# dRaniwal/RAJNI-ViT

Hardware: AMD Instinct MI355X
Metric: images/sec ViT-B/16@224 with README schedule (higher is better)
Workload: dtype bf16

## Files before the change

### rajni-vit_amd/csrc/attention.hip

```cpp
#include "common.h"

namespace {

constexpr int AT_THREADS = 256;
constexpr int AT_QROWS = 128;
constexpr int KV_CHUNK = 128;
constexpr int AT_LDS = 2 * KV_CHUNK * 128;

struct AttnArgs {
  const bf16_t* qkv;
  const int* idx;
  bf16_t* out;
  int n_src, np, H;
  int nq;
  float c;
  unsigned long long* stamps;
  unsigned char* out8;
  float oinv, oscale;
  float* row_scale;
};
__device__ __forceinline__ unsigned attn_pack4_e4m3(float a, float b, float c, float d) {
  a = __builtin_amdgcn_fmed3f(a, -448.f, 448.f); b = __builtin_amdgcn_fmed3f(b, -448.f, 448.f);
  c = __builtin_amdgcn_fmed3f(c, -448.f, 448.f); d = __builtin_amdgcn_fmed3f(d, -448.f, 448.f);
  int r = __builtin_amdgcn_cvt_pk_fp8_f32(a, b, 0, false);
  r = __builtin_amdgcn_cvt_pk_fp8_f32(c, d, r, true);
  return (unsigned)r;
}

__device__ __forceinline__ int k_off(int row, int chunk) {
  return row * 128 + ((chunk ^ ((row >> 1) & 7)) << 4);
}
__device__ __forceinline__ int v_off(int row, int chunk) {
  return row * 128 + ((chunk ^ (((row >> 1) & 1) << 2)) << 4);
}

__device__ __forceinline__ bf16x8 tr_pair(const char* sv, int row, int col) {
  typedef __attribute__((address_space(3))) s16x4* lds_s16x4;
  const int o0 = v_off(row, col >> 3) + (col & 7) * 2;
  const int o1 = v_off(row + 8, col >> 3) + (col & 7) * 2;
  const s16x4 lo = __builtin_amdgcn_ds_read_tr16_b64_v4i16((lds_s16x4)(sv + o0));
  const s16x4 hi = __builtin_amdgcn_ds_read_tr16_b64_v4i16((lds_s16x4)(sv + o1));
  typedef __attribute__((ext_vector_type(8))) short s16x8;
  const s16x8 v = {lo[0], lo[1], lo[2], lo[3], hi[0], hi[1], hi[2], hi[3]};
  return __builtin_bit_cast(bf16x8, v);
}

template <typename A = bf16_t>
__global__ void __launch_bounds__(AT_THREADS) attn_bf16_d64(const AttnArgs a) {
  __shared__ __attribute__((aligned(16))) char smem[AT_LDS];
  char* sk = smem;
  char* sv = smem + KV_CHUNK * 128;
  const int tid = threadIdx.x, wave = tid >> 6, lane = tid & 63;
  const int l31 = lane & 31, h = lane >> 5, g = lane >> 4, l15 = lane & 15;
  const int head = blockIdx.y, b = blockIdx.z;
  const int np = a.np, C = a.H * 64, C3 = 3 * C;
  const bf16_t* img = a.qkv + (long)b * a.n_src * C3;
  const int* idx = a.idx ? a.idx + (long)b * np : nullptr;

  const int qbase = blockIdx.x * AT_QROWS + wave * 32;
  const bool active = qbase < (a.nq < np ? a.nq : np);

  bf16x8 qf[4];
  {
    int q = qbase + l31;
    if (q > np - 1) q = np - 1;
    const int srow = idx ? idx[q] : q;
    const bf16_t* qp = img + (long)srow * C3 + head * 64 + 8 * h;
#pragma unroll
    for (int s = 0; s < 4; ++s) qf[s] = *reinterpret_cast<const bf16x8*>(qp + 16 * s);
  }

  f32x16 o0, o1;
#pragma unroll
  for (int r = 0; r < 16; ++r) { o0[r] = 0.f; o1[r] = 0.f; }
  float m_run = -INFINITY, l_run = 0.f;

  const int st_c = tid & 7, st_r = tid >> 3;

  for (int c0 = 0; c0 < np; c0 += KV_CHUNK) {
    uint4 kreg[4], vreg[4];
#pragma unroll
    for (int i = 0; i < 4; ++i) {
      const int t = c0 + st_r + 32 * i;
      if (t < np) {
        const int srow = idx ? idx[t] : t;
        const bf16_t* rp = img + (long)srow * C3 + head * 64 + st_c * 8;
        kreg[i] = *reinterpret_cast<const uint4*>(rp + C);
        vreg[i] = *reinterpret_cast<const uint4*>(rp + 2 * C);
      } else {
        kreg[i] = make_uint4(0, 0, 0, 0);
        vreg[i] = make_uint4(0, 0, 0, 0);
      }
    }
    __syncthreads();
#pragma unroll
    for (int i = 0; i < 4; ++i) {
      const int row = st_r + 32 * i;
      *reinterpret_cast<uint4*>(sk + k_off(row, st_c)) = kreg[i];
      *reinterpret_cast<uint4*>(sv + v_off(row, st_c)) = vreg[i];
    }
    __syncthreads();

    if (active) {
      const int nsub = (np - c0 + 31) >> 5;
      for (int kb = 0; kb < 4 && kb < nsub; ++kb) {
        f32x16 s;
#pragma unroll
        for (int r = 0; r < 16; ++r) s[r] = 0.f;
        const int krow = kb * 32 + l31;
#pragma unroll
        for (int ks = 0; ks < 4; ++ks) {
          const bf16x8 kf = *reinterpret_cast<const bf16x8*>(sk + k_off(krow, 2 * ks + h));
          s = mfma_32x32x16<A>(kf, qf[ks], s);
        }
        const int nvalid = np - c0 - kb * 32;
        if (nvalid < 32) {
#pragma unroll
          for (int r = 0; r < 16; ++r) {
            const int kr = (r & 3) + 8 * (r >> 2) + 4 * h;
            if (kr >= nvalid) s[r] = -INFINITY;
          }
        }
        float mx = s[0];
#pragma unroll
        for (int r = 1; r < 16; ++r) mx = fmaxf(mx, s[r]);
        mx = fmaxf(mx, __shfl_xor(mx, 32, 64));
        const float mxc = mx * a.c;
        if (__builtin_amdgcn_ballot_w64(mxc > m_run + 8.0f) != 0) {
          const float m_new = fmaxf(m_run, mxc);
          const float alpha = __builtin_amdgcn_exp2f(m_run - m_new);
          l_run *= alpha;
          m_run = m_new;
#pragma unroll
          for (int r = 0; r < 16; ++r) { o0[r] *= alpha; o1[r] *= alpha; }
        }
        float p[16];
        float lsum = 0.f;
#pragma unroll
        for (int r = 0; r < 16; ++r) {
          p[r] = __builtin_amdgcn_exp2f(fmaf(s[r], a.c, -m_run));
          lsum += p[r];
        }
        l_run += lsum;
        bf16x8 pb[2];
#pragma unroll
        for (int s2 = 0; s2 < 2; ++s2) {
          typedef __attribute__((ext_vector_type(4))) unsigned u32x4;
          const u32x4 w = {pack2<A>(p[8 * s2 + 0], p[8 * s2 + 1]), pack2<A>(p[8 * s2 + 2], p[8 * s2 + 3]),
                           pack2<A>(p[8 * s2 + 4], p[8 * s2 + 5]), pack2<A>(p[8 * s2 + 6], p[8 * s2 + 7])};
          pb[s2] = __builtin_bit_cast(bf16x8, w);
        }
#pragma unroll
        for (int s2 = 0; s2 < 2; ++s2) {
          const int key0 = kb * 32 + 16 * s2 + 4 * h + (l15 >> 2);
          const int col = 16 * (g & 1) + 4 * (l15 & 3);
          const bf16x8 v0 = tr_pair(sv, key0, col);
          const bf16x8 v1 = tr_pair(sv, key0, 32 + col);
          o0 = mfma_32x32x16<A>(v0, pb[s2], o0);
          o1 = mfma_32x32x16<A>(v1, pb[s2], o1);
        }
      }
    }
  }

  if (!active) return;
  const float l_tot = l_run + __shfl_xor(l_run, 32, 64);
  const float inv = 1.0f / l_tot;
  const int q = qbase + l31;
  if (q < np) {
    bf16_t* op = a.out + ((long)b * np + q) * C + head * 64 + 4 * h;
#pragma unroll
    for (int t = 0; t < 4; ++t) {
      uint2 w0, w1;
      w0.x = pack2<A>(o0[4 * t] * inv, o0[4 * t + 1] * inv);
      w0.y = pack2<A>(o0[4 * t + 2] * inv, o0[4 * t + 3] * inv);
      w1.x = pack2<A>(o1[4 * t] * inv, o1[4 * t + 1] * inv);
      w1.y = pack2<A>(o1[4 * t + 2] * inv, o1[4 * t + 3] * inv);
      *reinterpret_cast<uint2*>(op + 8 * t) = w0;
      *reinterpret_cast<uint2*>(op + 32 + 8 * t) = w1;
    }
  }
}


constexpr int ATF_THREADS = 512;
#ifndef RAJNI_ATTN_STAGE_MASK
#define RAJNI_ATTN_STAGE_MASK 0x78
#endif
constexpr bool stage_o(int nsub) { return (RAJNI_ATTN_STAGE_MASK >> (nsub - 1)) & 1; }

template <typename A, int NSUB, bool O8 = false>
__device__ __forceinline__ void attn_tile_compute(const char* sk, const char* sv, const bf16x8 (&qf)[4],
                                                  const AttnArgs& a, int b, int head, int qbase, int lane,
                                                  char* so = nullptr) {
  const int l31 = lane & 31, h = lane >> 5, g = lane >> 4, l15 = lane & 15;
  const int np = a.np, C = a.H * 64;
  f32x16 s[NSUB];
#pragma unroll
  for (int kb = 0; kb < NSUB; ++kb) {
#pragma unroll
    for (int r = 0; r < 16; ++r) s[kb][r] = 0.f;
    const int krow = kb * 32 + l31;
#pragma unroll
    for (int ks = 0; ks < 4; ++ks) {
      const bf16x8 kf = *reinterpret_cast<const bf16x8*>(sk + k_off(krow, 2 * ks + h));
      s[kb] = mfma_32x32x16<A>(kf, qf[ks], s[kb]);
    }
  }
#ifdef RAJNI_ATTN_STAMPS
  asm volatile("" :: "v"(s[0][0]), "v"(s[NSUB - 1][15]));
  const unsigned long long tsS = __builtin_amdgcn_s_memtime();
#endif
  {
    const int nvalid = np - (NSUB - 1) * 32;
    if (nvalid < 32) {
#pragma unroll
      for (int r = 0; r < 16; ++r) {
        const int kr = (r & 3) + 8 * (r >> 2) + 4 * h;
        if (kr >= nvalid) s[NSUB - 1][r] = -INFINITY;
      }
    }
  }
  float mx = s[0][0];
#pragma unroll
  for (int kb = 0; kb < NSUB; ++kb)
#pragma unroll
    for (int r = 0; r < 16; ++r) mx = fmaxf(mx, s[kb][r]);
  mx = fmaxf(mx, __shfl_xor(mx, 32, 64));
  const float mc = mx * a.c;
  float lsum = 0.f;
  f32x16 o0, o1;
#pragma unroll
  for (int r = 0; r < 16; ++r) { o0[r] = 0.f; o1[r] = 0.f; }
#pragma unroll
  for (int kb = 0; kb < NSUB; ++kb) {
    float p[16];
#pragma unroll
    for (int r = 0; r < 16; ++r) {
      p[r] = __builtin_amdgcn_exp2f(fmaf(s[kb][r], a.c, -mc));
      lsum += p[r];
    }
    bf16x8 pb[2];
#pragma unroll
    for (int s2 = 0; s2 < 2; ++s2) {
      typedef __attribute__((ext_vector_type(4))) unsigned u32x4;
      const u32x4 w = {pack2<A>(p[8 * s2 + 0], p[8 * s2 + 1]), pack2<A>(p[8 * s2 + 2], p[8 * s2 + 3]),
                       pack2<A>(p[8 * s2 + 4], p[8 * s2 + 5]), pack2<A>(p[8 * s2 + 6], p[8 * s2 + 7])};
      pb[s2] = __builtin_bit_cast(bf16x8, w);
    }
#pragma unroll
    for (int s2 = 0; s2 < 2; ++s2) {
      const int key0 = kb * 32 + 16 * s2 + 4 * h + (l15 >> 2);
      const int col = 16 * (g & 1) + 4 * (l15 & 3);
      const bf16x8 v0 = tr_pair(sv, key0, col);
      const bf16x8 v1 = tr_pair(sv, key0, 32 + col);
      o0 = mfma_32x32x16<A>(v0, pb[s2], o0);
      o1 = mfma_32x32x16<A>(v1, pb[s2], o1);
    }
  }
#ifdef RAJNI_ATTN_STAMPS
  asm volatile("" :: "v"(o0[0]), "v"(o1[15]));
  const unsigned long long tsP = __builtin_amdgcn_s_memtime();
  if (a.stamps != nullptr && qbase == 0 && lane == 0) {
    unsigned long long* o = a.stamps + ((size_t)b * a.H + head) * 8;
    o[1] = tsS; o[2] = tsP;
  }
#endif
  const float inv = 1.0f / (lsum + __shfl_xor(lsum, 32, 64));
  const int q = qbase + l31;
  __builtin_amdgcn_s_waitcnt(0x0F70);
  if constexpr (O8) {
    const float sc = inv * a.oinv;
    const int key = (l31 >> 2) & 3;
    char* wr = so + l31 * 64 + 4 * (h & 1);
#pragma unroll
    for (int t = 0; t < 4; ++t) {
      const unsigned w0 = attn_pack4_e4m3(o0[4 * t] * sc, o0[4 * t + 1] * sc, o0[4 * t + 2] * sc, o0[4 * t + 3] * sc);
      const unsigned w1 = attn_pack4_e4m3(o1[4 * t] * sc, o1[4 * t + 1] * sc, o1[4 * t + 2] * sc, o1[4 * t + 3] * sc);
      *reinterpret_cast<unsigned*>(wr + (((t >> 1) ^ key) << 4) + 8 * (t & 1)) = w0;
      *reinterpret_cast<unsigned*>(wr + (((2 + (t >> 1)) ^ key) << 4) + 8 * (t & 1)) = w1;
    }
    __builtin_amdgcn_fence(__ATOMIC_RELEASE, "wavefront");
    __builtin_amdgcn_wave_barrier();
    const int u = lane & 3;
    unsigned char* ob = a.out8 + ((long)b * np + qbase) * C + head * 64 + u * 16;
#pragma unroll
    for (int j = 0; j < 2; ++j) {
      const int r = (lane >> 2) + 16 * j;
      const uint4 v = *reinterpret_cast<const uint4*>(so + r * 64 + ((u ^ ((r >> 2) & 3)) << 4));
      if (qbase + r < np) *reinterpret_cast<uint4*>(ob + (long)r * C) = v;
    }
    if (head == 0 && h == 0 && q < np) a.row_scale[(long)b * np + q] = a.oscale;
    return;
  }
  if (so != nullptr) {
    const int key = (l31 ^ (l31 >> 3)) & 7;
    char* wr = so + l31 * 128 + 8 * h;
#pragma unroll
    for (int t = 0; t < 4; ++t) {
      uint2 w0, w1;
      w0.x = pack2<A>(o0[4 * t] * inv, o0[4 * t + 1] * inv);
      w0.y = pack2<A>(o0[4 * t + 2] * inv, o0[4 * t + 3] * inv);
      w1.x = pack2<A>(o1[4 * t] * inv, o1[4 * t + 1] * inv);
      w1.y = pack2<A>(o1[4 * t + 2] * inv, o1[4 * t + 3] * inv);
      *reinterpret_cast<uint2*>(wr + ((t ^ key) << 4)) = w0;
      *reinterpret_cast<uint2*>(wr + (((4 + t) ^ key) << 4)) = w1;
    }
    const int u = lane & 7;
    bf16_t* ob = a.out + ((long)b * np + qbase) * C + head * 64 + u * 8;
#pragma unroll
    for (int j = 0; j < 4; ++j) {
      const int r = (lane >> 3) + 8 * j;
      const uint4 v = *reinterpret_cast<const uint4*>(so + r * 128 + ((u ^ ((r ^ (r >> 3)) & 7)) << 4));
      if (qbase + r < np) *reinterpret_cast<uint4*>(ob + (long)r * C) = v;
    }
    return;
  }
  if (q < np) {
    bf16_t* op = a.out + ((long)b * np + q) * C + head * 64 + 4 * h;
#pragma unroll
    for (int t = 0; t < 4; ++t) {
      uint2 w0, w1;
      w0.x = pack2<A>(o0[4 * t] * inv, o0[4 * t + 1] * inv);
      w0.y = pack2<A>(o0[4 * t + 2] * inv, o0[4 * t + 3] * inv);
      w1.x = pack2<A>(o1[4 * t] * inv, o1[4 * t + 1] * inv);
      w1.y = pack2<A>(o1[4 * t + 2] * inv, o1[4 * t + 3] * inv);
      *reinterpret_cast<uint2*>(op + 8 * t) = w0;
      *reinterpret_cast<uint2*>(op + 32 + 8 * t) = w1;
    }
  }
}

template <int NSUB, typename A = bf16_t>
__global__ void __launch_bounds__(ATF_THREADS, 2) attn_bf16_d64_full(const AttnArgs a) {
  extern __shared__ __attribute__((aligned(16))) char smem[];
  constexpr int ROWS = NSUB * 32;
  char* sk = smem;
  char* sv = smem + ROWS * 128;
  const int tid = threadIdx.x, wave = tid >> 6, lane = tid & 63;
  const int l31 = lane & 31, h = lane >> 5, g = lane >> 4, l15 = lane & 15;
  const int head = blockIdx.x, b = blockIdx.y;
  const int np = a.np, C = a.H * 64, C3 = 3 * C;
  const bf16_t* img = a.qkv + (long)b * a.n_src * C3;
  const int* idx = a.idx ? a.idx + (long)b * np : nullptr;
  const int qbase = wave * 32;
  const bool active = qbase < (a.nq < np ? a.nq : np);

  bf16x8 qf[4];
  {
    int q = qbase + l31;
    if (q > np - 1) q = np - 1;
    const int srow = idx ? idx[q] : q;
    const bf16_t* qp = img + (long)srow * C3 + head * 64 + 8 * h;
#pragma unroll
    for (int s = 0; s < 4; ++s) qf[s] = *reinterpret_cast<const bf16x8*>(qp + 16 * s);
  }
  {
    const int st_c = tid & 7, st_r = tid >> 3;
#pragma unroll
    for (int i = 0; i < (ROWS + 63) / 64; ++i) {
      const int t = st_r + 64 * i;
      if (t < ROWS) {
        uint4 kr = make_uint4(0, 0, 0, 0), vr = make_uint4(0, 0, 0, 0);
        if (t < np) {
          const int srow = idx ? idx[t] : t;
          const bf16_t* rp = img + (long)srow * C3 + head * 64 + st_c * 8;
          kr = *reinterpret_cast<const uint4*>(rp + C);
          vr = *reinterpret_cast<const uint4*>(rp + 2 * C);
        }
        *reinterpret_cast<uint4*>(sk + k_off(t, st_c)) = kr;
        *reinterpret_cast<uint4*>(sv + v_off(t, st_c)) = vr;
      }
    }
  }
  __syncthreads();
  if (!active) return;
  attn_tile_compute<A, NSUB>(sk, sv, qf, a, b, head, qbase, lane);
}

__device__ __forceinline__ void dma16(const char* base, unsigned off, char* dst) {
  const unsigned lds = __builtin_amdgcn_readfirstlane((unsigned)(size_t)LDS_PTR(dst));
  unsigned keep;
  asm volatile("s_mov_b32 %0, m0\n\ts_mov_b32 m0, %2\n\ts_nop 0\n\tglobal_load_lds_dwordx4 %1, %3\n\ts_mov_b32 m0, %0"
               : "=&s"(keep) : "v"(off), "s"(lds), "s"(base) : "memory");
}

template <int NSUB, bool G, bool O8 = false, typename A = bf16_t>
__global__ void __launch_bounds__(ATF_THREADS, 2) attn_bf16_d64_stream(const AttnArgs a, int n_items) {
  extern __shared__ __attribute__((aligned(16))) char smem[];
  constexpr int ROWS = NSUB * 32, BUF = ROWS * 256, NP8 = ROWS / 8;
  constexpr bool STAGE_O = O8 || stage_o(NSUB);
  constexpr int STAGE_BYTES = O8 ? 2048 : 4096;
  constexpr int PER_WAVE = (NP8 + 7) / 8;
  const int tid = threadIdx.x, lane = tid & 63;
  const int wave = __builtin_amdgcn_readfirstlane(tid >> 6);
  const int l31 = lane & 31, h = lane >> 5;
  const int np = a.np, C = a.H * 64, C3 = 3 * C;
  const int qbase = wave * 32;
  const bool active = qbase < (a.nq < np ? a.nq : np);
  const int r_in = lane >> 3, pos = lane & 7;

  int trow[PER_WAVE];
#pragma unroll
  for (int i = 0; i < PER_WAVE; ++i) {
    const int t = (wave + 8 * i) * 8 + r_in;
    trow[i] = t < np ? t : np - 1;
  }
  const int tq = qbase + l31 < np ? qbase + l31 : np - 1;

  const unsigned ck = (unsigned)(pos ^ ((4 * (wave & 1) + (r_in >> 1)) & 7)) << 4;
  const unsigned cv = (unsigned)(pos ^ (((r_in >> 1) & 1) << 2)) << 4;
  const unsigned row_bytes = (unsigned)C3 * 2;

  auto load_rows = [&](int b, int (&srow)[PER_WAVE], int& sq) {
    if constexpr (G) {
      const int* idx = a.idx + (long)b * np;
#pragma unroll
      for (int i = 0; i < PER_WAVE; ++i) srow[i] = idx[trow[i]];
      sq = idx[tq];
    } else {
#pragma unroll
      for (int i = 0; i < PER_WAVE; ++i) srow[i] = trow[i];
      sq = tq;
    }
  };
  auto dma_item = [&](int b, int head, const int (&srow)[PER_WAVE], int buf) {
    const char* bk = reinterpret_cast<const char*>(a.qkv) + ((size_t)b * a.n_src * C3 + head * 64 + C) * 2;
    const char* bv = bk + (size_t)C * 2;
    char* sk = smem + buf * BUF;
    char* sv = sk + ROWS * 128;
#pragma unroll
    for (int i = 0; i < PER_WAVE; ++i) {
      const int q = wave + 8 * i;
      if (q < NP8) {
        const unsigned ro = (unsigned)srow[i] * row_bytes;
        dma16(bk, ro + ck, sk + q * 1024);
        dma16(bv, ro + cv, sv + q * 1024);
      }
    }
  };
  auto load_q = [&](int b, int head, int sq, bf16x8 (&qf)[4]) {
    const char* bq = reinterpret_cast<const char*>(a.qkv) + ((size_t)b * a.n_src * C3 + head * 64) * 2;
    const unsigned qo = (unsigned)sq * row_bytes + 16 * h;
#pragma unroll
    for (int s = 0; s < 4; ++s) qf[s] = *reinterpret_cast<const bf16x8*>(bq + (size_t)(qo + 32 * s));
  };

  int item = blockIdx.x;
  if (item >= n_items) return;
  int srow_a[PER_WAVE], sq_a;
  bf16x8 qf[4], qn[4];
  int cb = item / a.H, chead = item - cb * a.H;
  load_rows(cb, srow_a, sq_a);
  dma_item(cb, chead, srow_a, 0);
  load_q(cb, chead, sq_a, qn);
  int nxt = item + gridDim.x;
  load_rows((nxt < n_items ? nxt : n_items - 1) / a.H, srow_a, sq_a);
  int buf = 0;
  __builtin_amdgcn_s_waitcnt(0x0F70);
  while (true) {
    if (!active) __builtin_amdgcn_s_waitcnt(0x0F70);
    asm volatile("s_waitcnt lgkmcnt(0)" ::: "memory");
#ifdef RAJNI_ATTN_STAMPS
    const unsigned long long ts_arrive = __builtin_amdgcn_s_memtime();
#endif
    __builtin_amdgcn_s_barrier();
#ifdef RAJNI_ATTN_STAMPS
    const unsigned long long ts_bar = __builtin_amdgcn_s_memtime();
#endif
    asm volatile("" ::: "memory");
#pragma unroll
    for (int s = 0; s < 4; ++s) { asm volatile("" : "+v"(qn[s])); qf[s] = qn[s]; }
#pragma unroll
    for (int i = 0; i < PER_WAVE; ++i) asm volatile("" : "+v"(srow_a[i]));
    asm volatile("" : "+v"(sq_a));
    const int last = n_items - 1;
    const int nx = nxt < last ? nxt : last;
    const int nn = nxt + (int)gridDim.x < last ? nxt + (int)gridDim.x : last;
    int srow_use[PER_WAVE];
#pragma unroll
    for (int i = 0; i < PER_WAVE; ++i) srow_use[i] = srow_a[i];
    const int nb = nx / a.H, nhead = nx - nb * a.H;
    load_q(nb, nhead, sq_a, qn);
    load_rows(nn / a.H, srow_a, sq_a);
    dma_item(nb, nhead, srow_use, buf ^ 1);
#ifdef RAJNI_ATTN_STAMPS
    const unsigned long long ts_issue = __builtin_amdgcn_s_memtime();
#endif
    if (active) {
      const int b = cb, head = chead;
      attn_tile_compute<A, NSUB, O8>(smem + buf * BUF, smem + buf * BUF + ROWS * 128, qf, a, b, head, qbase, lane,
                                  STAGE_O ? smem + 2 * BUF + (qbase >> 5) * STAGE_BYTES : nullptr);
    }
#ifdef RAJNI_ATTN_STAMPS
    if (a.stamps != nullptr && qbase == 0 && lane == 0) {
      unsigned long long* o = a.stamps + (size_t)item * 8;
      o[0] = ts_arrive; o[3] = ts_bar; o[4] = ts_issue; o[5] = __builtin_amdgcn_s_memtime();
    }
#endif
    if (nxt >= n_items) break;
    item = nxt;
    cb = nb; chead = nhead;
    nxt += gridDim.x;
    buf ^= 1;
  }
  asm volatile("s_waitcnt vmcnt(0)" ::: "memory");
}

struct AttnArgsF32 {
  const float* qkv; const int* idx; float* out;
  int n_src, np, H;
  float c;
  int nq;
};

__global__ void __launch_bounds__(256) attn_f32_d64(const AttnArgsF32 a) {
  __shared__ __attribute__((aligned(16))) float sk[64 * 64];
  __shared__ __attribute__((aligned(16))) float sv[64 * 64];
  const int tid = threadIdx.x;
  const int qrow = tid >> 2, pt = tid & 3;
  const int head = blockIdx.y, b = blockIdx.z;
  const int np = a.np, C = a.H * 64, C3 = 3 * C;
  const float* img = a.qkv + (long)b * a.n_src * C3;
  const int* idx = a.idx ? a.idx + (long)b * np : nullptr;
  int q = blockIdx.x * 64 + qrow;
  const bool valid = q < np;
  if (!valid) q = np - 1;
  float qv[16], o[16];
  {
    const int srow = idx ? idx[q] : q;
    const float* qp = img + (long)srow * C3 + head * 64 + pt * 16;
#pragma unroll
    for (int j = 0; j < 4; ++j) {
      const float4 t = reinterpret_cast<const float4*>(qp)[j];
      qv[4 * j] = t.x; qv[4 * j + 1] = t.y; qv[4 * j + 2] = t.z; qv[4 * j + 3] = t.w;
    }
  }
#pragma unroll
  for (int j = 0; j < 16; ++j) o[j] = 0.f;
  float m_run = -INFINITY, l_run = 0.f;
  for (int c0 = 0; c0 < np; c0 += 64) {
    __syncthreads();
#pragma unroll
    for (int i = 0; i < 4; ++i) {
      const int e = tid + 256 * i;
      const int r = e >> 4, c4 = e & 15;
      const int t = c0 + r;
      float4 kq = make_float4(0, 0, 0, 0), vq = make_float4(0, 0, 0, 0);
      if (t < np) {
        const int srow = idx ? idx[t] : t;
        const float* rp = img + (long)srow * C3 + head * 64 + c4 * 4;
        kq = *reinterpret_cast<const float4*>(rp + C);
        vq = *reinterpret_cast<const float4*>(rp + 2 * C);
      }
      reinterpret_cast<float4*>(sk)[e] = kq;
      reinterpret_cast<float4*>(sv)[e] = vq;
    }
    __syncthreads();
    const int nk = np - c0 < 64 ? np - c0 : 64;
    for (int j = 0; j < nk; ++j) {
      const float* kr = sk + j * 64 + pt * 16;
      float d = 0.f;
#pragma unroll
      for (int e = 0; e < 16; ++e) d = fmaf(qv[e], kr[e], d);
      d += __shfl_xor(d, 1, 64);
      d += __shfl_xor(d, 2, 64);
      const float sc = d * a.c;
      const float m_new = fmaxf(m_run, sc);
      const float alpha = __builtin_amdgcn_exp2f(m_run - m_new);
      const float pj = __builtin_amdgcn_exp2f(sc - m_new);
      l_run = fmaf(l_run, alpha, pj);
      m_run = m_new;
      const float* vr = sv + j * 64 + pt * 16;
#pragma unroll
      for (int e = 0; e < 16; ++e) o[e] = fmaf(o[e], alpha, pj * vr[e]);
    }
  }
  if (valid) {
    const float inv = 1.0f / l_run;
    float* op = a.out + ((long)b * np + q) * C + head * 64 + pt * 16;
#pragma unroll
    for (int j = 0; j < 4; ++j)
      reinterpret_cast<float4*>(op)[j] = make_float4(o[4 * j] * inv, o[4 * j + 1] * inv, o[4 * j + 2] * inv, o[4 * j + 3] * inv);
  }
}


constexpr int AG_KSTRIDE = 136;
constexpr int AG_VSTRIDE = 68;
constexpr int AG_QROWS = 128;
typedef __attribute__((ext_vector_type(4))) short s16x4_t;

template <int NW, int NB, typename A = bf16_t>
__global__ void __launch_bounds__(NW * 64, 2) attn_bf16_dgen(const AttnArgs a, int D) {
  constexpr int NT = NW * 64, QROWS = NW * NB * 16, KI = 1024 / NT;
  __shared__ __attribute__((aligned(16))) bf16_t sk[64 * AG_KSTRIDE];
  __shared__ __attribute__((aligned(16))) bf16_t svt[128 * AG_VSTRIDE];
  const int tid = threadIdx.x, wave = tid >> 6, lane = tid & 63;
  const int r = lane & 15, g = lane >> 4;
  const int head = blockIdx.y, b = blockIdx.z;
  const int np = a.np, C = a.H * D, C3 = 3 * C;
  const int ND = (D + 15) >> 4;
  const bf16_t* img = a.qkv + (long)b * a.n_src * C3 + head * D;
  const int* idx = a.idx ? a.idx + (long)b * np : nullptr;

  int q[NB];
  bool valid[NB];
  s16x4_t qf[NB][8];
#pragma unroll
  for (int u = 0; u < NB; ++u) {
    q[u] = blockIdx.x * QROWS + (wave * NB + u) * 16 + r;
    valid[u] = q[u] < np;
    if (!valid[u]) q[u] = np - 1;
    const int srow = idx ? idx[q[u]] : q[u];
    const bf16_t* qp = img + (long)srow * C3;
#pragma unroll
    for (int kd = 0; kd < 8; ++kd) {
      qf[u][kd] = s16x4_t{0, 0, 0, 0};
      const int d0 = 16 * kd + 4 * g;
      if (kd < ND && d0 < D) qf[u][kd] = *reinterpret_cast<const s16x4_t*>(qp + d0);
    }
  }
  f32x4 o[NB][8];
#pragma unroll
  for (int u = 0; u < NB; ++u)
#pragma unroll
    for (int db = 0; db < 8; ++db) o[u][db] = f32x4{0.f, 0.f, 0.f, 0.f};
  float m_run[NB], l_part[NB];
#pragma unroll
  for (int u = 0; u < NB; ++u) { m_run[u] = -INFINITY; l_part[u] = 0.f; }
  const int chunks8 = 2 * ND;

  uint4 kreg[KI], vreg[4];
  const int n_kitems = 64 * chunks8, n_vitems = 16 * chunks8;
  auto fetch = [&](int c0) {
#pragma unroll
    for (int i = 0; i < KI; ++i) {
      const int item = tid + NT * i;
      kreg[i] = make_uint4(0, 0, 0, 0);
      if (item < n_kitems) {
        const int row = item / chunks8, d0 = (item - row * chunks8) * 8;
        const int t = c0 + row;
        if (t < np && d0 < D) {
          const int srow = idx ? idx[t] : t;
          kreg[i] = *reinterpret_cast<const uint4*>(img + (long)srow * C3 + C + d0);
        }
      }
    }
    if (tid < n_vitems) {
      const int r4 = tid / chunks8, d0 = (tid - r4 * chunks8) * 8;
#pragma unroll
      for (int i = 0; i < 4; ++i) {
        const int t = c0 + 4 * r4 + i;
        vreg[i] = make_uint4(0, 0, 0, 0);
        if (t < np && d0 < D) {
          const int srow = idx ? idx[t] : t;
          vreg[i] = *reinterpret_cast<const uint4*>(img + (long)srow * C3 + 2 * C + d0);
        }
      }
    }
  };
  fetch(0);

  for (int c0 = 0; c0 < np; c0 += 64) {
    __syncthreads();
#pragma unroll
    for (int i = 0; i < KI; ++i) {
      const int item = tid + NT * i;
      if (item < n_kitems) {
        const int row = item / chunks8, d0 = (item - row * chunks8) * 8;
        *reinterpret_cast<uint4*>(sk + row * AG_KSTRIDE + d0) = kreg[i];
      }
    }
    if (tid < n_vitems) {
      const int r4 = tid / chunks8, d0 = (tid - r4 * chunks8) * 8;
      const unsigned w[4][4] = {{vreg[0].x, vreg[0].y, vreg[0].z, vreg[0].w}, {vreg[1].x, vreg[1].y, vreg[1].z, vreg[1].w},
                                {vreg[2].x, vreg[2].y, vreg[2].z, vreg[2].w}, {vreg[3].x, vreg[3].y, vreg[3].z, vreg[3].w}};
#pragma unroll
      for (int j = 0; j < 8; ++j) {
        unsigned e[4];
#pragma unroll
        for (int i = 0; i < 4; ++i) e[i] = (j & 1) ? (w[i][j >> 1] >> 16) : (w[i][j >> 1] & 0xFFFFu);
        *reinterpret_cast<uint2*>(svt + (d0 + j) * AG_VSTRIDE + 4 * r4) = make_uint2(e[0] | (e[1] << 16), e[2] | (e[3] << 16));
      }
    }
    __syncthreads();
    if (c0 + 64 < np) fetch(c0 + 64);

    f32x4 st[NB][4];
    float mloc[NB];
#pragma unroll
    for (int u = 0; u < NB; ++u) mloc[u] = -INFINITY;
#pragma unroll
    for (int kb = 0; kb < 4; ++kb) {
#pragma unroll
      for (int u = 0; u < NB; ++u) st[u][kb] = f32x4{0.f, 0.f, 0.f, 0.f};
#pragma unroll
      for (int kd = 0; kd < 8; ++kd)
        if (kd < ND) {
          const s16x4_t ka = *reinterpret_cast<const s16x4_t*>(sk + (16 * kb + r) * AG_KSTRIDE + 16 * kd + 4 * g);
#pragma unroll
          for (int u = 0; u < NB; ++u) st[u][kb] = mfma_16x16x16<A>(ka, qf[u][kd], st[u][kb]);
        }
#pragma unroll
      for (int u = 0; u < NB; ++u)
#pragma unroll
        for (int j = 0; j < 4; ++j) {
          const int key = c0 + 16 * kb + 4 * g + j;
          const float v = key < np ? st[u][kb][j] * a.c : -INFINITY;
          st[u][kb][j] = v;
          mloc[u] = fmaxf(mloc[u], v);
        }
    }
    float alpha[NB];
    s16x4_t pf[NB][4];
#pragma unroll
    for (int u = 0; u < NB; ++u) {
      float ml = fmaxf(mloc[u], __shfl_xor(mloc[u], 16, 64));
      ml = fmaxf(ml, __shfl_xor(ml, 32, 64));
      const float m_new = fmaxf(m_run[u], ml);
      alpha[u] = __builtin_amdgcn_exp2f(m_run[u] - m_new);
      m_run[u] = m_new;
      float psum = 0.f;
#pragma unroll
      for (int kb = 0; kb < 4; ++kb) {
        float pv[4];
#pragma unroll
        for (int j = 0; j < 4; ++j) {
          pv[j] = __builtin_amdgcn_exp2f(st[u][kb][j] - m_new);
          psum += pv[j];
        }
        pf[u][kb] = __builtin_bit_cast(s16x4_t, make_uint2(pack2<A>(pv[0], pv[1]), pack2<A>(pv[2], pv[3])));
      }
      l_part[u] = fmaf(l_part[u], alpha[u], psum);
    }
#pragma unroll
    for (int db = 0; db < 8; ++db)
      if (db < ND) {
#pragma unroll
        for (int u = 0; u < NB; ++u) o[u][db] *= alpha[u];
#pragma unroll
        for (int kb = 0; kb < 4; ++kb) {
          const s16x4_t va = *reinterpret_cast<const s16x4_t*>(svt + (16 * db + r) * AG_VSTRIDE + 16 * kb + 4 * g);
#pragma unroll
          for (int u = 0; u < NB; ++u) o[u][db] = mfma_16x16x16<A>(va, pf[u][kb], o[u][db]);
        }
      }
  }
#pragma unroll
  for (int u = 0; u < NB; ++u) {
    float l = l_part[u] + __shfl_xor(l_part[u], 16, 64);
    l += __shfl_xor(l, 32, 64);
    if (valid[u]) {
      const float inv = 1.0f / l;
      bf16_t* op = a.out + ((long)b * np + q[u]) * C + head * D;
#pragma unroll
      for (int db = 0; db < 8; ++db) {
        const int d0 = 16 * db + 4 * g;
        if (db < ND && d0 < D)
          *reinterpret_cast<uint2*>(op + d0) =
              make_uint2(pack2<A>(o[u][db][0] * inv, o[u][db][1] * inv), pack2<A>(o[u][db][2] * inv, o[u][db][3] * inv));
      }
    }
  }
}

template <int DQM>
__global__ void __launch_bounds__(256) attn_f32_dgen(const AttnArgsF32 a, int D) {
  __shared__ __attribute__((aligned(16))) float sk[32 * 4 * DQM];
  __shared__ __attribute__((aligned(16))) float sv[32 * 4 * DQM];
  const int tid = threadIdx.x;
  const int qrow = tid >> 2, pt = tid & 3;
  const int head = blockIdx.y, b = blockIdx.z;
  const int np = a.np, C = a.H * D, C3 = 3 * C, DQ = D >> 2, D4 = D >> 2;
  const float* img = a.qkv + (long)b * a.n_src * C3 + head * D;
  const int* idx = a.idx ? a.idx + (long)b * np : nullptr;
  int q = blockIdx.x * 64 + qrow;
  const bool valid = q < np;
  if (!valid) q = np - 1;
  float qv[DQM], o[DQM];
  {
    const int srow = idx ? idx[q] : q;
    const float* qp = img + (long)srow * C3 + pt * DQ;
#pragma unroll
    for (int e = 0; e < DQM; ++e) {
      qv[e] = e < DQ ? qp[e] : 0.f;
      o[e] = 0.f;
    }
  }
  float m_run = -INFINITY, l_run = 0.f;
  for (int c0 = 0; c0 < np; c0 += 32) {
    __syncthreads();
    for (int e = tid; e < 32 * D4; e += 256) {
      const int row = e / D4, c4 = e - row * D4;
      const int t = c0 + row;
      float4 kq = make_float4(0, 0, 0, 0), vq = make_float4(0, 0, 0, 0);
      if (t < np) {
        const int srow = idx ? idx[t] : t;
        const float* rp = img + (long)srow * C3 + c4 * 4;
        kq = *reinterpret_cast<const float4*>(rp + C);
        vq = *reinterpret_cast<const float4*>(rp + 2 * C);
      }
      reinterpret_cast<float4*>(sk)[e] = kq;
      reinterpret_cast<float4*>(sv)[e] = vq;
    }
    __syncthreads();
    const int nk = np - c0 < 32 ? np - c0 : 32;
    for (int j = 0; j < nk; ++j) {
      const float* kr = sk + j * D + pt * DQ;
      float d = 0.f;
#pragma unroll
      for (int e = 0; e < DQM; ++e)
        if (e < DQ) d = fmaf(qv[e], kr[e], d);
      d += __shfl_xor(d, 1, 64);
      d += __shfl_xor(d, 2, 64);
      const float sc = d * a.c;
      const float m_new = fmaxf(m_run, sc);
      const float alpha = __builtin_amdgcn_exp2f(m_run - m_new);
      const float pj = __builtin_amdgcn_exp2f(sc - m_new);
      l_run = fmaf(l_run, alpha, pj);
      m_run = m_new;
      const float* vr = sv + j * D + pt * DQ;
#pragma unroll
      for (int e = 0; e < DQM; ++e)
        if (e < DQ) o[e] = fmaf(o[e], alpha, pj * vr[e]);
    }
  }
  if (valid) {
    const float inv = 1.0f / l_run;
    float* op = a.out + ((long)b * np + q) * C + head * D + pt * DQ;
#pragma unroll
    for (int e = 0; e < DQM; ++e)
      if (e < DQ) op[e] = o[e] * inv;
  }
}

int g_force_attn = 0;

template <int NSUB>
int launch_full_o8(const AttnArgs& a, int B, hipStream_t s) {
  constexpr int lds = NSUB * 32 * 256 * 2 + 8 * 2048;
  static bool attr_by_device[RAJNI_MAX_DEVICES] = {};
  bool& attr = attr_by_device[rajni_current_device()];
  if (!attr && lds > 64 * 1024) {
    for (const void* fn : {reinterpret_cast<const void*>(&attn_bf16_d64_stream<NSUB, false, true>),
                           reinterpret_cast<const void*>(&attn_bf16_d64_stream<NSUB, true, true>)}) {
      hipError_t e = hipFuncSetAttribute(fn, hipFuncAttributeMaxDynamicSharedMemorySize, lds);
      if (e != hipSuccess) { rajni_set_error("hipFuncSetAttribute(attn): %s", hipGetErrorString(e)); return RAJNI_ERR_LAUNCH; }
    }
    attr = true;
  }
  const int per_cu = (160 * 1024) / lds >= 2 ? 2 : 1;
  const int items = a.H * B;
  const int cus = rajni_num_cus();
  const int grid = rajni_persistent_grid(items < cus * per_cu ? items : cus * per_cu);
  if (a.idx != nullptr)
    hipLaunchKernelGGL((attn_bf16_d64_stream<NSUB, true, true>), dim3(grid), dim3(ATF_THREADS), lds, s, a, items);
  else
    hipLaunchKernelGGL((attn_bf16_d64_stream<NSUB, false, true>), dim3(grid), dim3(ATF_THREADS), lds, s, a, items);
  return RAJNI_OK;
}

template <int NSUB, typename A>
int launch_full(const AttnArgs& a, int B, hipStream_t s) {
  if (g_force_attn == 2) {
    constexpr int lds = NSUB * 32 * 128 * 2;
    hipLaunchKernelGGL((attn_bf16_d64_full<NSUB, A>), dim3(a.H, B), dim3(ATF_THREADS), lds, s, a);
    return RAJNI_OK;
  }
  constexpr int lds = NSUB * 32 * 256 * 2 + (stage_o(NSUB) ? 8 * 4096 : 0);
  static bool attr_by_device[RAJNI_MAX_DEVICES] = {};
  bool& attr = attr_by_device[rajni_current_device()];
  if (!attr && lds > 64 * 1024) {
    for (const void* fn : {reinterpret_cast<const void*>(&attn_bf16_d64_stream<NSUB, false, false, A>),
                           reinterpret_cast<const void*>(&attn_bf16_d64_stream<NSUB, true, false, A>)}) {
      hipError_t e = hipFuncSetAttribute(fn, hipFuncAttributeMaxDynamicSharedMemorySize, lds);
      if (e != hipSuccess) { rajni_set_error("hipFuncSetAttribute(attn): %s", hipGetErrorString(e)); return RAJNI_ERR_LAUNCH; }
    }
    attr = true;
  }
  const int per_cu = (160 * 1024) / lds >= 2 ? 2 : 1;
  const int items = a.H * B;
  const int cus = rajni_num_cus();
  const int grid = rajni_persistent_grid(items < cus * per_cu ? items : cus * per_cu);
  if (a.idx != nullptr)
    hipLaunchKernelGGL((attn_bf16_d64_stream<NSUB, true, false, A>), dim3(grid), dim3(ATF_THREADS), lds, s, a, items);
  else
    hipLaunchKernelGGL((attn_bf16_d64_stream<NSUB, false, false, A>), dim3(grid), dim3(ATF_THREADS), lds, s, a, items);
  return RAJNI_OK;
}

}

template <typename T>
__global__ void __launch_bounds__(64) attn_cls_kernel(const T* qkv, T* out, int N, int H, int D, float c, float q_scale) {
  extern __shared__ __attribute__((aligned(16))) float cls_sm[];
  float* qs = cls_sm;
  float* prob = cls_sm + D;
  const int lane = threadIdx.x, head = blockIdx.x, b = blockIdx.y;
  const int C = H * D, C3 = 3 * C;
  const T* img = qkv + (long)b * N * C3 + head * D;
  for (int d = lane; d < D; d += 64) qs[d] = ld1(img + d);
  __syncthreads();
  float mx = -INFINITY;
  for (int n = lane; n < N; n += 64) {
    const T* kr = img + (long)n * C3 + C;
    float dot = 0.f;
    for (int i = 0; i < (D >> 3); ++i) {
      float kf[8];
      load8<T>(kr + 8 * i, kf);
#pragma unroll
      for (int j = 0; j < 8; ++j) dot = fmaf(qs[8 * i + j], kf[j], dot);
    }
    dot *= c;
    prob[n] = dot;
    mx = fmaxf(mx, dot);
  }
  mx = wave_max(mx);
  float sum = 0.f;
  for (int n = lane; n < N; n += 64) {
    const float pr = __builtin_amdgcn_exp2f(prob[n] - mx);
    prob[n] = pr;
    sum += pr;
  }
  sum = wave_sum(sum);
  __syncthreads();
  for (int d = lane; d < D; d += 64) {
    float acc = 0.f;
    const T* vc = img + 2 * C + d;
    for (int n = 0; n < N; ++n) acc = fmaf(prob[n], ld1(vc + (long)n * C3), acc);
    float o = acc / sum;
    if (q_scale > 0.f) {
      const float t = __builtin_amdgcn_fmed3f(o * (1.0f / q_scale), -448.f, 448.f);
      o = __builtin_amdgcn_cvt_f32_fp8(__builtin_amdgcn_cvt_pk_fp8_f32(t, 0.f, 0, false), 0) * q_scale;
    }
    st1(out + (long)b * C + head * D + d, o);
  }
}

int launch_attention_cls(const void* qkv, void* out, int B, int N, int H, int D, float scale, int dtype,
                         hipStream_t s, float q_scale) {
  RAJNI_REQUIRE(qkv && out && D >= 8 && D <= 128 && D % 8 == 0 && B > 0 && H > 0 && N > 0 && B <= 65535 &&
                (size_t)(N + D) * sizeof(float) <= 64 * 1024, RAJNI_ERR_INVALID, "attention_cls: bad arguments");
  const float c = scale * 1.4426950408889634f;
  const size_t lds = (size_t)(N + D) * sizeof(float);
  ProfScope prof(KC_ATTENTION, s, 4.0 * B * H * (double)N * D, 2.0 * B * (double)N * H * D * (dtype == RAJNI_F32 ? 4.0 : 2.0));
  if (dtype == RAJNI_F32)
    hipLaunchKernelGGL(attn_cls_kernel<float>, dim3(H, B), dim3(64), lds, s, (const float*)qkv, (float*)out, N, H, D, c, 0.f);
  else if (dtype == RAJNI_F16)
    hipLaunchKernelGGL(attn_cls_kernel<f16_t>, dim3(H, B), dim3(64), lds, s, (const f16_t*)qkv, (f16_t*)out, N, H, D, c, 0.f);
  else
    hipLaunchKernelGGL(attn_cls_kernel<bf16_t>, dim3(H, B), dim3(64), lds, s, (const bf16_t*)qkv, (bf16_t*)out, N, H, D, c, q_scale);
  RAJNI_CHECK_LAUNCH("attn_cls_kernel");
  return RAJNI_OK;
}

template <typename A>
int launch_attention16(const AttnArgs& a, int B, int np, int H, int D, hipStream_t s) {
  const int nsub = (np + 31) / 32;
  if (D != 64) {
    #ifndef RAJNI_ATTN_DGEN_NW
#define RAJNI_ATTN_DGEN_NW 4
#endif
#ifndef RAJNI_ATTN_DGEN_NB
#define RAJNI_ATTN_DGEN_NB 2
#endif
    constexpr int qrows = RAJNI_ATTN_DGEN_NW * RAJNI_ATTN_DGEN_NB * 16;
    hipLaunchKernelGGL((attn_bf16_dgen<RAJNI_ATTN_DGEN_NW, RAJNI_ATTN_DGEN_NB, A>), dim3((a.nq + qrows - 1) / qrows, H, B),
                       dim3(RAJNI_ATTN_DGEN_NW * 64), 0, s, a, D);
  } else if (nsub <= 8 && g_force_attn != 1) {
    int rc = RAJNI_OK;
    switch (nsub) {
      case 1: rc = launch_full<1, A>(a, B, s); break;
      case 2: rc = launch_full<2, A>(a, B, s); break;
      case 3: rc = launch_full<3, A>(a, B, s); break;
      case 4: rc = launch_full<4, A>(a, B, s); break;
      case 5: rc = launch_full<5, A>(a, B, s); break;
      case 6: rc = launch_full<6, A>(a, B, s); break;
      case 7: rc = launch_full<7, A>(a, B, s); break;
      default: rc = launch_full<8, A>(a, B, s); break;
    }
    if (rc != RAJNI_OK) return rc;
  } else {
    hipLaunchKernelGGL(attn_bf16_d64<A>, dim3((a.nq + AT_QROWS - 1) / AT_QROWS, H, B), dim3(AT_THREADS), 0,
                       s, a);
  }
  return RAJNI_OK;
}

static inline bool image_bytes_ok(int n_src, int H) { return (size_t)n_src * 3 * (size_t)H * 64 * 2 <= 0xFFFFFFFFul; }

int launch_attention(const void* qkv, const int32_t* keep_idx, void* out, int B, int n_src, int np, int nq,
                     int H, int D, float scale, int dtype, hipStream_t s) {
  RAJNI_REQUIRE(H <= RAJNI_MAX_GRID_YZ && B <= RAJNI_MAX_GRID_YZ, RAJNI_ERR_UNSUPPORTED,
                "rajni_attention: B=%d H=%d - one launch takes at most %d images and %d heads (grid y / z)", B, H,
                RAJNI_MAX_GRID_YZ, RAJNI_MAX_GRID_YZ);
  const bool persistent = D == 64 && dtype != RAJNI_F32 && (np + 31) / 32 <= 8 && g_force_attn == 0;
  RAJNI_REQUIRE(!persistent || image_bytes_ok(n_src, H), RAJNI_ERR_UNSUPPORTED,
                "rajni_attention: one image of qkv is n_src=%d x 3*H*64 x 2 bytes - with up to 256 kept tokens the limit is 2^32 - 1 "
                "bytes per image", n_src);
  RAJNI_REQUIRE(qkv && out, RAJNI_ERR_INVALID, "rajni_attention: null pointer");
  RAJNI_REQUIRE(D >= 8 && D <= 128 && D % 8 == 0, RAJNI_ERR_UNSUPPORTED,
                "rajni_attention: head dim %d not supported (multiples of 8 up to 128)", D);
  RAJNI_REQUIRE(B > 0 && H > 0 && np > 0 && n_src >= np, RAJNI_ERR_INVALID,
                "rajni_attention: bad shape B=%d H=%d np=%d n_src=%d", B, H, np, n_src);
  RAJNI_REQUIRE(keep_idx != nullptr || np == n_src, RAJNI_ERR_INVALID,
                "rajni_attention: identity selection needs np == n_src");
  RAJNI_REQUIRE(nq >= 1 && nq <= np, RAJNI_ERR_INVALID, "rajni_attention: query-row limit nq=%d outside 1..np=%d", nq, np);
  const double kv_q_o = 2.0 * np + 2.0 * nq;
  if (dtype == RAJNI_F32) {
    AttnArgsF32 f{};
    f.qkv = (const float*)qkv; f.idx = keep_idx; f.out = (float*)out;
    f.n_src = n_src; f.np = np; f.H = H; f.c = scale * 1.4426950408889634f; f.nq = nq;
    ProfScope prof(KC_ATTENTION, s, 4.0 * B * H * (double)nq * np * D, 4.0 * B * kv_q_o * H * D);
    const dim3 grid((nq + 63) / 64, H, B);
    if (D == 64) hipLaunchKernelGGL(attn_f32_d64, grid, dim3(256), 0, s, f);
    else if (D < 64) hipLaunchKernelGGL(attn_f32_dgen<16>, grid, dim3(256), 0, s, f, D);
    else hipLaunchKernelGGL(attn_f32_dgen<32>, grid, dim3(256), 0, s, f, D);
    RAJNI_CHECK_LAUNCH("attn_f32");
    return RAJNI_OK;
  }
  RAJNI_REQUIRE(dtype == RAJNI_BF16 || dtype == RAJNI_F16, RAJNI_ERR_INVALID, "rajni_attention: bad dtype %d", dtype);
  AttnArgs a{};
  a.qkv = (const bf16_t*)qkv; a.idx = keep_idx; a.out = (bf16_t*)out;
  a.n_src = n_src; a.np = np; a.H = H; a.nq = nq;
  a.c = scale * 1.4426950408889634f;
  a.stamps = rajni_g_stamps;
  const double flops = 4.0 * B * H * (double)nq * np * D;
  const double bytes = 2.0 * B * kv_q_o * H * D;
  ProfScope prof(KC_ATTENTION, s, flops, bytes);
  const int rc = dtype == RAJNI_F16 ? launch_attention16<f16_t>(a, B, np, H, D, s) : launch_attention16<bf16_t>(a, B, np, H, D, s);
  if (rc != RAJNI_OK) return rc;
  RAJNI_CHECK_LAUNCH("attn_bf16_d64");
  return RAJNI_OK;
}

int launch_attention_fp8(const void* qkv, const int32_t* keep_idx, void* out_q, float out_scale, float* row_scale,
                         int B, int n_src, int np, int H, int D, float scale, hipStream_t s) {
  RAJNI_REQUIRE(H <= RAJNI_MAX_GRID_YZ && B <= RAJNI_MAX_GRID_YZ, RAJNI_ERR_UNSUPPORTED,
                "rajni_attention_fp8: B=%d H=%d - one launch takes at most %d images and %d heads", B, H, RAJNI_MAX_GRID_YZ,
                RAJNI_MAX_GRID_YZ);
  RAJNI_REQUIRE(image_bytes_ok(n_src, H), RAJNI_ERR_UNSUPPORTED,
                "rajni_attention_fp8: one image of qkv is n_src=%d x 3*H*64 x 2 bytes - the limit is 2^32 - 1 bytes per image", n_src);
  RAJNI_REQUIRE(qkv && out_q && row_scale, RAJNI_ERR_INVALID, "rajni_attention_fp8: null pointer");
  RAJNI_REQUIRE(D == 64 && np <= 224, RAJNI_ERR_UNSUPPORTED,
                "rajni_attention_fp8: head dim 64 and at most 224 tokens (D=%d np=%d)", D, np);
  RAJNI_REQUIRE(B > 0 && H > 0 && np > 0 && n_src >= np, RAJNI_ERR_INVALID,
                "rajni_attention_fp8: bad shape B=%d H=%d np=%d n_src=%d", B, H, np, n_src);
  RAJNI_REQUIRE(keep_idx != nullptr || np == n_src, RAJNI_ERR_INVALID,
                "rajni_attention_fp8: identity selection needs np == n_src");
  RAJNI_REQUIRE(out_scale > 0.f && out_scale < INFINITY, RAJNI_ERR_INVALID, "rajni_attention_fp8: out_scale must be positive and finite");
  AttnArgs a{};
  a.qkv = (const bf16_t*)qkv; a.idx = keep_idx; a.out = nullptr;
  a.n_src = n_src; a.np = np; a.H = H; a.nq = np;
  a.c = scale * 1.4426950408889634f;
  a.stamps = nullptr;
  a.out8 = (unsigned char*)out_q; a.oscale = out_scale; a.oinv = 1.0f / out_scale; a.row_scale = row_scale;
  ProfScope prof(KC_ATTENTION, s, 4.0 * B * H * (double)np * np * D, 2.0 * B * (double)np * H * D * 3.5);
  int rc = RAJNI_OK;
  switch ((np + 31) / 32) {
    case 1: rc = launch_full_o8<1>(a, B, s); break;
    case 2: rc = launch_full_o8<2>(a, B, s); break;
    case 3: rc = launch_full_o8<3>(a, B, s); break;
    case 4: rc = launch_full_o8<4>(a, B, s); break;
    case 5: rc = launch_full_o8<5>(a, B, s); break;
    case 6: rc = launch_full_o8<6>(a, B, s); break;
    default: rc = launch_full_o8<7>(a, B, s); break;
  }
  if (rc != RAJNI_OK) return rc;
  RAJNI_CHECK_LAUNCH("attn_bf16_d64_stream<e4m3 out>");
  return RAJNI_OK;
}

extern "C" void rajni_debug_force_attention(int mode) { g_force_attn = mode; }
```

Baseline: 30220.

## Split stream attention waves into dedicated K/V DMA producers and compute consumers

For persistent attention kernels with fewer than 8 query subtiles, the waves that have no query rows now act as producers. They prefetch the next item's K/V into a double-buffered LDS slot through direct global-to-LDS loads while the active waves compute the current tile. The consumer waves also prefetch the next item's Q fragments and gather indices into registers. This replaces the uniform load-then-compute loop with a warp-specialized pipeline synchronized per item by a workgroup barrier. It risks load imbalance, because fewer waves issue the DMA and the barrier couples the two roles.

```diff
diff --git a/rajni-vit_amd/csrc/attention.hip b/rajni-vit_amd/csrc/attention.hip
--- a/rajni-vit_amd/csrc/attention.hip
+++ b/rajni-vit_amd/csrc/attention.hip
@@ -378,16 +378,185 @@
   attn_tile_compute<A, NSUB>(sk, sv, qf, a, b, head, qbase, lane);
 }
 
-__device__ __forceinline__ void dma16(const char* base, unsigned off, char* dst) {
-  const unsigned lds = __builtin_amdgcn_readfirstlane((unsigned)(size_t)LDS_PTR(dst));
+__device__ __forceinline__ void dma16_at(const char* base, unsigned off, unsigned lds) {
   unsigned keep;
   asm volatile("s_mov_b32 %0, m0\n\ts_mov_b32 m0, %2\n\ts_nop 0\n\tglobal_load_lds_dwordx4 %1, %3\n\ts_mov_b32 m0, %0"
                : "=&s"(keep) : "v"(off), "s"(lds), "s"(base) : "memory");
 }
+__device__ __forceinline__ void dma16(const char* base, unsigned off, char* dst) {
+  dma16_at(base, off, __builtin_amdgcn_readfirstlane((unsigned)(size_t)LDS_PTR(dst)));
+}
+
+#ifndef RAJNI_ATTN_ROLE_MASK
+#define RAJNI_ATTN_ROLE_MASK 0x7F
+#endif
+constexpr bool role_split(int nsub) { return nsub < 8 && ((RAJNI_ATTN_ROLE_MASK >> (nsub - 1)) & 1); }
+
+template <int NSUB, bool G, bool O8, typename A>
+__device__ __forceinline__ void attn_stream_roles(const AttnArgs& a, const int n_items, char* smem) {
+  constexpr int ROWS = NSUB * 32, BUF = ROWS * 256, NP8 = ROWS / 8;
+  constexpr bool STAGE_O = O8 || stage_o(NSUB);
+  constexpr int STAGE_BYTES = O8 ? 2048 : 4096;
+  constexpr int PP_MAX = (NP8 + (8 - NSUB) - 1) / (8 - NSUB);
+  const int tid = threadIdx.x, lane = tid & 63;
+  const int wave = __builtin_amdgcn_readfirstlane(tid >> 6);
+  const int np = a.np, H = a.H, C = H * 64, C3 = 3 * C;
+  const unsigned row_bytes = (unsigned)C3 * 2;
+  const int nact = ((a.nq < np ? a.nq : np) + 31) >> 5;
+
+  int item = blockIdx.x;
+  if (item >= n_items) return;
+  const int step = (int)gridDim.x, last = n_items - 1;
+  const int dB = step / H, dH = step - dB * H;
+  const int lb = last / H, lhead = last - lb * H;
+  auto advance = [&](int& b, int& head) {
+    b += dB; head += dH;
+    if (head >= H) { head -= H; ++b; }
+  };
+  int cb = item / H, chead = item - cb * H;
+  int b1 = cb, h1 = chead;
+  advance(b1, h1);
+  int b2 = b1, h2 = h1;
+  advance(b2, h2);
+  int nxt = item + step;
+  int buf = 0;
+
+  if (wave >= nact) {
+    auto produce = [&](auto full) __attribute__((always_inline)) {
+    constexpr bool FULL = decltype(full)::value;
+    const int nprod = FULL ? 8 - NSUB : 8 - nact;
+    const int p = FULL && NSUB == 7 ? 0 : wave - nact;
+    __builtin_assume(p >= 0 && p < nprod);
+    const int r_in = lane >> 3, pos = lane & 7;
+    const unsigned ck0 = (unsigned)(pos ^ (r_in >> 1)) << 4;
+    const unsigned cv = (unsigned)(pos ^ (((r_in >> 1) & 1) << 2)) << 4;
+    const unsigned lds0 = __builtin_amdgcn_readfirstlane((unsigned)(size_t)LDS_PTR(smem));
+    auto load_rows = [&](int b, int (&srow)[PP_MAX]) {
+      const int* idx = G ? a.idx + (long)b * np : nullptr;
+#pragma unroll
+      for (int i = 0; i < PP_MAX; ++i) {
+        const int q = p + nprod * i;
+        if (q < NP8) {
+          const int t = q * 8 + r_in;
+          const int tr = t < np ? t : np - 1;
+          if constexpr (G) srow[i] = idx[tr]; else srow[i] = tr;
+        }
+      }
+    };
+    auto dma_item = [&](int b, int head, const int (&srow)[PP_MAX], int to) {
+      const char* bk = reinterpret_cast<const char*>(a.qkv) + ((size_t)b * a.n_src * C3 + head * 64 + C) * 2;
+      const char* bv = bk + (size_t)C * 2;
+      const unsigned sk = lds0 + to * BUF, sv = sk + ROWS * 128;
+#pragma unroll
+      for (int i = 0; i < PP_MAX; ++i) {
+        const int q = p + nprod * i;
+        if (q < NP8) {
+          const unsigned ro = (unsigned)srow[i] * row_bytes;
+          dma16_at(bk, ro + (ck0 ^ ((unsigned)(q & 1) << 6)), __builtin_amdgcn_readfirstlane(sk + q * 1024));
+          dma16_at(bv, ro + cv, __builtin_amdgcn_readfirstlane(sv + q * 1024));
+        }
+      }
+    };
+    int srow_a[PP_MAX] = {}, srow_use[PP_MAX];
+    load_rows(cb, srow_a);
+    __builtin_amdgcn_s_waitcnt(0x0F70);
+    dma_item(cb, chead, srow_a, 0);
+    load_rows(nxt <= last ? b1 : lb, srow_a);
+    __builtin_amdgcn_s_waitcnt(0x0F70);
+    while (true) {
+      __builtin_amdgcn_s_barrier();
+#ifdef RAJNI_ATTN_STAMPS
+      const unsigned long long ts_bar = __builtin_amdgcn_s_memtime();
+#endif
+      const bool in1 = nxt <= last, in2 = nxt + step <= last;
+#pragma unroll
+      for (int i = 0; i < PP_MAX; ++i) srow_use[i] = srow_a[i];
+      load_rows(in2 ? b2 : lb, srow_a);
+      dma_item(in1 ? b1 : lb, in1 ? h1 : lhead, srow_use, buf ^ 1);
+#ifdef RAJNI_ATTN_STAMPS
+      const unsigned long long ts_issue = __builtin_amdgcn_s_memtime();
+#endif
+      __builtin_amdgcn_s_waitcnt(0x0F70);
+#ifdef RAJNI_ATTN_STAMPS
+      if (a.stamps != nullptr && p == 0 && lane == 0) {
+        unsigned long long* o = a.stamps + (size_t)item * 8;
+        o[6] = ts_issue - ts_bar; o[7] = __builtin_amdgcn_s_memtime() - ts_issue;
+      }
+#endif
+      if (nxt >= n_items) break;
+      item = nxt;
+      b1 = b2; h1 = h2;
+      advance(b2, h2);
+      nxt += step;
+      buf ^= 1;
+    }
+    };
+    if (nact == NSUB) produce(std::true_type{});
+    else produce(std::false_type{});
+    return;
+  }
+  const int l31 = lane & 31, h = lane >> 5;
+  const int qbase = wave * 32;
+  const int tq = qbase + l31 < np ? qbase + l31 : np - 1;
+  auto load_sq = [&](int b) -> int {
+    if constexpr (G) return a.idx[(long)b * np + tq];
+    else return tq;
+  };
+  auto load_q = [&](int b, int head, int sq, bf16x8 (&qf)[4]) {
+    const char* bq = reinterpret_cast<const char*>(a.qkv) + ((size_t)b * a.n_src * C3 + head * 64) * 2;
+    const unsigned qo = (unsigned)sq * row_bytes + 16 * h;
+#pragma unroll
+    for (int s = 0; s < 4; ++s) qf[s] = *reinterpret_cast<const bf16x8*>(bq + (size_t)(qo + 32 * s));
+  };
+  bf16x8 qf[4], qn[4];
+  int sq_a = load_sq(cb);
+  load_q(cb, chead, sq_a, qn);
+  sq_a = load_sq(nxt <= last ? b1 : lb);
+  __builtin_amdgcn_s_waitcnt(0x0F70);
+  while (true) {
+    asm volatile("s_waitcnt lgkmcnt(0)" ::: "memory");
+#ifdef RAJNI_ATTN_STAMPS
+    const unsigned long long ts_arrive = __builtin_amdgcn_s_memtime();
+#endif
+    __builtin_amdgcn_s_barrier();
+#ifdef RAJNI_ATTN_STAMPS
+    const unsigned long long ts_bar = __builtin_amdgcn_s_memtime();
+#endif
+    asm volatile("" ::: "memory");
+#pragma unroll
+    for (int s = 0; s < 4; ++s) { asm volatile("" : "+v"(qn[s])); qf[s] = qn[s]; }
+    asm volatile("" : "+v"(sq_a));
+    const bool in1 = nxt <= last, in2 = nxt + step <= last;
+    load_q(in1 ? b1 : lb, in1 ? h1 : lhead, sq_a, qn);
+    sq_a = load_sq(in2 ? b2 : lb);
+#ifdef RAJNI_ATTN_STAMPS
+    const unsigned long long ts_issue = __builtin_amdgcn_s_memtime();
+#endif
+    attn_tile_compute<A, NSUB, O8>(smem + buf * BUF, smem + buf * BUF + ROWS * 128, qf, a, cb, chead, qbase, lane,
+                                   STAGE_O ? smem + 2 * BUF + (qbase >> 5) * STAGE_BYTES : nullptr);
+#ifdef RAJNI_ATTN_STAMPS
+    if (a.stamps != nullptr && qbase == 0 && lane == 0) {
+      unsigned long long* o = a.stamps + (size_t)item * 8;
+      o[0] = ts_arrive; o[3] = ts_bar; o[4] = ts_issue; o[5] = __builtin_amdgcn_s_memtime();
+    }
+#endif
+    if (nxt >= n_items) break;
+    item = nxt;
+    cb = b1; chead = h1;
+    b1 = b2; h1 = h2;
+    advance(b2, h2);
+    nxt += step;
+    buf ^= 1;
+  }
+}
 
 template <int NSUB, bool G, bool O8 = false, typename A = bf16_t>
 __global__ void __launch_bounds__(ATF_THREADS, 2) attn_bf16_d64_stream(const AttnArgs a, int n_items) {
   extern __shared__ __attribute__((aligned(16))) char smem[];
+  if constexpr (role_split(NSUB)) {
+    attn_stream_roles<NSUB, G, O8, A>(a, n_items, smem);
+    return;
+  }
   constexpr int ROWS = NSUB * 32, BUF = ROWS * 256, NP8 = ROWS / 8;
   constexpr bool STAGE_O = O8 || stage_o(NSUB);
   constexpr int STAGE_BYTES = O8 ? 2048 : 4096;
```

Result: no change. 30380 (median of 6 runs) (+0.5%).
